# tum-vision/lsd_slam

Measured on AMD Instinct MI355X. Metric: tracked frames/sec (full track+map loop) at 640x480, frames resident in HBM (8-bit upload excluded: value_pcie_inclusive has it), higher is better.
Workload: dtype f32

## Files before the change

lsd_slam_amd/csrc/track_device.hpp:

```cpp
#pragma once
#include "lsdhip_internal.hpp"
#include <type_traits>

template <int CTRL, int ROW_MASK, int BANK_MASK>
__device__ __forceinline__ float dpp_f(float v) {
  return __builtin_bit_cast(float, __builtin_amdgcn_update_dpp(0, __builtin_bit_cast(int, v), CTRL, ROW_MASK, BANK_MASK, true));
}
__device__ __forceinline__ int dpp_max_i(int a, int b) { return a > b ? a : b; }
template <int CTRL, int ROW_MASK, int BANK_MASK>
__device__ __forceinline__ int dpp_i(int v) {
  return __builtin_amdgcn_update_dpp(-1, v, CTRL, ROW_MASK, BANK_MASK, false);
}
template <int CTRL, int ROW_MASK, int BANK_MASK>
__device__ __forceinline__ int dpp_i0(int v) {
  return __builtin_amdgcn_update_dpp(0, v, CTRL, ROW_MASK, BANK_MASK, true);
}
__device__ __forceinline__ int wave_max_to_lane63(int v) {
  int t = dpp_max_i(v, dpp_i<0x111, 0xf, 0xf>(v));
  t = dpp_max_i(t, dpp_i<0x112, 0xf, 0xf>(v));
  t = dpp_max_i(t, dpp_i<0x113, 0xf, 0xf>(v));
  t = dpp_max_i(t, dpp_i<0x114, 0xf, 0xe>(t));
  t = dpp_max_i(t, dpp_i<0x118, 0xf, 0xc>(t));
  t = dpp_max_i(t, dpp_i<0x142, 0xa, 0xf>(t));
  t = dpp_max_i(t, dpp_i<0x143, 0xc, 0xf>(t));
// ... 553 lines not shown
  } else {
    S.level = S.level - 1;
    S.phase = 0;
    set_eval_pose(S, T);
  }
  return false;
}

__device__ __forceinline__ void accumulate_point(const PointOut& o, float (&acc)[RS_END]) {
  acc[RS_M] += 1.f;
  acc[RS_SXX] = __builtin_fmaf(o.c1 * o.c1, o.hw, acc[RS_SXX]);
  acc[RS_SYY] = __builtin_fmaf(o.c2 * o.c2, o.hw, acc[RS_SYY]);
  acc[RS_SX] = __builtin_fmaf(o.c1, o.hw, acc[RS_SX]);
  acc[RS_SY] = __builtin_fmaf(o.c2, o.hw, acc[RS_SY]);
  acc[RS_SW] += o.hw;
  if (o.good) { acc[RS_GOOD] += 1.f; acc[RS_SUMRES2] = __builtin_fmaf(o.res, o.res, acc[RS_SUMRES2]); acc[RS_SUMSIGNED] += o.res; }
  else acc[RS_BAD] += 1.f;
  acc[RS_USAGE] += o.usage;
  acc[RS_WERR] += o.werr;
#pragma unroll
  for (int r = 0; r < 6; r++) {
    float Jw = o.J[r] * o.w;
#pragma unroll
    for (int c = r; c < 6; c++) acc[tri_index(r, c)] = __builtin_fmaf(Jw, o.J[c], acc[tri_index(r, c)]);
  }
  float resw = o.res * o.w;
#pragma unroll
  for (int r = 0; r < 6; r++) acc[RS_B0 + r] = __builtin_fmaf(resw, o.J[r], acc[RS_B0 + r]);
  acc[RS_ERR] = __builtin_fmaf(resw, o.res, acc[RS_ERR]);
}

__device__ __forceinline__ void visit_point(const EvalCtx& a, const PointWarp& q, const PointTexels& t, const float pz, const float I_ref, const float var,
                                            gbyte* mask, const int maskIdx, const int key, float (&acc)[RS_END], int& key0, int& key1, int& key2) {
  acc[RS_NREF] += 1.f;
  if (!q.in_image) { if (mask) mask[maskIdx] = 0; return; }
  PointOut o;
  eval_finish(a, q, t, pz, I_ref, var, o);
  if (mask) mask[maskIdx] = o.good ? 1 : 0;
  top3_insert(key, key0, key1, key2);
  accumulate_point(o, acc);
}

enum { TAIL_WORDS = 29, TAIL_KEY = 31, TAIL_STRIDE = 32, TAIL_ROWS = 3 };
__device__ __forceinline__ void tail_row(const PointOut& o, float* row) {
  row[0] = o.werr;
  int k = 1;
#pragma unroll
  for (int rr = 0; rr < 6; rr++) {
    const float Jw = o.J[rr] * o.w;
#pragma unroll
    for (int cc = rr; cc < 6; cc++) row[k++] = Jw * o.J[cc];
  }
  const float resw = o.res * o.w;
#pragma unroll
  for (int rr = 0; rr < 6; rr++) row[k++] = resw * o.J[rr];
  row[k++] = resw * o.res;
}
__device__ __forceinline__ void tail_row_from_sums(const float (&acc)[RS_END], float* row) {
  row[0] = acc[RS_WERR];
#pragma unroll
  for (int k = 0; k < 21; k++) row[1 + k] = acc[RS_A0 + k];
#pragma unroll
  for (int k = 0; k < 6; k++) row[22 + k] = acc[RS_B0 + k];
  row[28] = acc[RS_ERR];
}
__device__ __forceinline__ int tail_word(const int col) {
  return (col == RS_WERR) ? 0 : ((col >= RS_A0 && col < RS_B0) ? 1 + col - RS_A0 : ((col >= RS_B0 && col < RS_ERR) ? 22 + col - RS_B0 : (col == RS_ERR ? 28 : -1)));
}
__device__ __forceinline__ float tail_drop(float s, const int M, const int nsub, const int word, const float (*sub)[TAIL_STRIDE]) {
  int need = M & 3;
  if (need > nsub) need = nsub;
  const float sub0 = sub[0][word < 0 ? 0 : word], sub1 = sub[1][word < 0 ? 0 : word], sub2 = sub[2][word < 0 ? 0 : word];
  if (word >= 0) {
    if (need > 0) s -= sub0;
    if (need > 1) s -= sub1;
    if (need > 2) s -= sub2;
  }
  return s;
}

struct TailCandidate {
  int key = -1, x = 0, y = 0;
  float var = 0.f, id = 1.f, img = 0.f;
  __device__ __forceinline__ void request(const EvalCtx& a, const int k) {
    key = k;
    if (k < 0) return;
    x = k / a.h; y = k - x * a.h;
    const int ci = __mul24(y, a.w) + x;
    var = a.kf_idepthVar[ci]; id = a.kf_idepth[ci]; img = a.kf_image[ci];
  }
};

template <int STRIDE, int RRUN>
__device__ __forceinline__ float slice_sum(const float* s_red, const int k, const int slice) {
  const float* row = s_red + k * STRIDE;
  const int j0 = slice * RRUN;
  float v[RRUN];
#pragma unroll
  for (int j = 0; j < RRUN; j++) v[j] = row[j0 + j];
  float s = 0.f;
#pragma unroll
  for (int j = 0; j < RRUN; j++) s += (j0 + j < STRIDE - 1) ? v[j] : 0.f;
  return s;
}

template <class Posed>
__device__ __forceinline__ void ctx_set_pose(EvalCtx& a, const Posed& p) {
#pragma unroll
  for (int i = 0; i < 9; i++) a.R[i] = p.R[i];
#pragma unroll
  for (int i = 0; i < 3; i++) a.t[i] = p.t[i];
}
__device__ __forceinline__ void make_ctx_dev(const TrackJob& jobr, const TrackState& S, int level, EvalCtx& a) {
  const TrackJob* job = &jobr;
  const TrackLevel& L = job->lv[level];
  a.kf_idepth = (gfloat*)L.kf_idepth; a.kf_idepthVar = (gfloat*)L.kf_idepthVar; a.kf_image = (gfloat*)L.kf_image; a.fr_grad = (gfloat*)L.fr_grad;
  a.pts_pos = (gfloat*)L.pts_pos; a.pts_colvar = (gfloat*)L.pts_colvar; a.npts = L.npts; a.w = L.w; a.h = L.h;
  a.fx = L.fx; a.fy = L.fy; a.cx = L.cx; a.cy = L.cy; a.fxi = L.fxi; a.fyi = L.fyi; a.cxi = L.cxi; a.cyi = L.cyi;
  ctx_set_pose(a, S);
  a.aff_a = S.aff_a; a.aff_b = S.aff_b;
  a.cameraPixelNoise2 = job->cameraPixelNoise2; a.var_weight = job->var_weight; a.huber_half = job->huber_half;
}

template <int N>
__device__ __forceinline__ void copy_words(void* dst, const void* src, int tid, int nthreads) {
  const unsigned* s = (const unsigned*)src;
  unsigned* d = (unsigned*)dst;
  for (int i = tid; i < N; i += nthreads) d[i] = s[i];
}

__device__ __forceinline__ int xcd_tile(int b, int nb) { return (nb & 7) == 0 ? (b & 7) * (nb >> 3) + (b >> 3) : b; }


struct TrialRecord {
  float inc[6];
  float pose[7];
  float R[9], t[3];
  float pad_[7];
};
static_assert(sizeof(TrialRecord) == 128 && sizeof(lsdm::SE3fH) == sizeof(float[7]), "a trial record is 32 floats; its pose is a TrackState::Tn");
enum { TRIAL_RECORD_WORDS = offsetof(TrialRecord, pad_) / 4 };
__device__ __forceinline__ float trial_record_word(const TrackState& S, const int i) {
  constexpr int P = offsetof(TrialRecord, pose) / 4, R = offsetof(TrialRecord, R) / 4, T = offsetof(TrialRecord, t) / 4;
  return i < P ? S.inc[i] : (i < R ? ((const float*)&S.Tn)[i - P] : (i < T ? S.R[i - R] : S.t[i - T]));
}
__device__ __forceinline__ void trial_record_adopt(TrackState& S, const TrialRecord& rec, const int lane) {
  if (lane < 6) S.inc[lane] = rec.inc[lane];
  if (lane < 7) ((float*)&S.Tn)[lane] = rec.pose[lane];
  if (lane < 9) S.R[lane] = rec.R[lane];
  if (lane < 3) S.t[lane] = rec.t[lane];
}
__device__ __forceinline__ int trials_at(const TrackSpec& spec, const int level) { return (spec.specC > 1 && spec.trials[level] > 1) ? spec.trials[level] : 1; }

#define RS_COLS 44
struct TrackScratch {
  float* sums;
  int4* topkey;
  float* topval;
  int max_rows;
  int cmax;
  TrialRecord* recs;
#ifdef LSD_PHASE_TRACE
  unsigned long long* trace;
#endif
};
```

lsd_slam_amd/csrc/tracker.hip:

```cpp
#include <atomic>
#include <chrono>
#include "track_device.hpp"
#include "reposition_plan.hpp"

#ifdef LSD_PHASE_TRACE
#define PHASE_MARK(k) do { if (trOn_ && threadIdx.x == 0) tr_[k] = clock64(); } while (0)
#define LSD_TRACE_WORDS 32
#define TRACE_PARAMS , const bool trOn_, unsigned long long* const tr_
#define TRACE_ARGS , trOn_, tr_
#define TRACE_PUT(rec, who, k, v) do { if (trOn_ && threadIdx.x == (who)) (rec)[k] = (unsigned long long)(v); } while (0)
#define TRACE_LM_REC (trOn_ ? tr_ : nullptr)
__device__ __forceinline__ unsigned long long* trace_open(unsigned long long* trace, const bool mine, unsigned long long** s_trp) {
  if (!mine) return trace;
  const unsigned long long n = trace[0];
  trace[0] = n + 1;
  unsigned long long* tr_ = trace + 1 + (n % 4096) * LSD_TRACE_WORDS;
  for (int k = 0; k < LSD_TRACE_WORDS; k++) tr_[k] = 0;
  tr_[8] = wall_clock64();
  tr_[24] = (unsigned long long)gridDim.x; tr_[25] = (unsigned long long)gridDim.y;
  *s_trp = tr_;
  return tr_;
}
#else
#define PHASE_MARK(k) do { } while (0)
#define TRACE_PARAMS
#define TRACE_ARGS
#define TRACE_PUT(rec, who, k, v) do { } while (0)
#define TRACE_LM_REC nullptr
#endif

#ifdef LSD_DEVTOOLS
#define LAUNCH_LOG(exitCode, pendingIn, ncandIn, pcUsed) do { \
    if (!BATCH && MODE == TS_FUSED && blockIdx.x == 0 && threadIdx.x == 0 && spec.dbgLog && spec.seq != 0) { \
      int* lg_ = spec.dbgLog + ((spec.seq & 0xFFF) * 16); \
      lg_[0] = spec.seq; lg_[1] = (exitCode); lg_[2] = parity | (first << 1) | (spec.last << 2); lg_[3] = lvlIn_; lg_[4] = (pendingIn); lg_[5] = (ncandIn); \
      lg_[6] = (pcUsed); lg_[7] = S.level; lg_[8] = S.numEvaluations; lg_[9] = S.numLaunches; lg_[10] = S.done; lg_[11] = S.phase; lg_[12] = S.incTry; \
      lg_[13] = S.ncand; lg_[14] = S.pending; lg_[15] = numLaunchesIn_; } } while (0)
#else
#define LAUNCH_LOG(exitCode, pendingIn, ncandIn, pcUsed) do { } while (0)
#endif

enum { TS_FUSED = 0, TS_LM = 1, TS_EVAL = 2 };
__device__ __forceinline__ void track_state_begin(TrackState& S, const TrackJob& job, const int tid) {
  if (tid == 0) {
    S.T = job.T0;
    set_eval_pose(S, job.T0);
    S.aff_a = job.aff_a0; S.aff_b = job.aff_b0; S.aff_a_lastIt = job.aff_a0; S.aff_b_lastIt = job.aff_b0;
    S.lastErr = 0; S.LM_lambda = 0; S.last_residual = 0;
    S.level = job.topLevel; S.iteration = 0; S.incTry = 0; S.phase = 0; S.pending = 0;
    S.done = 0; S.diverged = 0; S.numEvaluations = 0; S.numWarpUpdates = 0;
    S.pointUsage = 0; S.goodCount = 0; S.badCount = 0; S.meanRes = 0;
    S.bytes = 0;
    for (int l = 0; l < LSD_LEVELS; l++) S.levelEvals[l] = 0;
    S.ncand = 1; S.lastCand = 0; S.numLaunches = 0;
  }
  if (tid < 36) S.A[tid] = 0;
  if (tid < 6) { S.b[tid] = 0; S.inc[tid] = 0; }
}

struct StepAddr {
  const float *sums_in, *topval_in;
  float *sums_out, *topval_out;
  const int4* topkey_in; int4* topkey_out;
  const TrialRecord* recs_in;
  TrialRecord* recs_out;
  int max_rows, cmax;
};
template <bool BATCH, int MODE>
__device__ __forceinline__ StepAddr step_addr(const TrackScratch& sc, const int parity) {
  const size_t rows = (size_t)sc.max_rows, cm = (size_t)sc.cmax, job0 = BATCH ? (size_t)blockIdx.y * 2 * cm : 0;
  const size_t in = job0 + (size_t)parity * cm, out = job0 + (size_t)(MODE == TS_EVAL ? parity : 1 - parity) * cm;
  constexpr size_t TAIL = TAIL_ROWS * TAIL_STRIDE;
  return {sc.sums + in * RS_COLS * rows, sc.topval + in * rows * TAIL, sc.sums + out * RS_COLS * rows, sc.topval + out * rows * TAIL,
          sc.topkey + in * rows, sc.topkey + out * rows, sc.recs + in, sc.recs + out, sc.max_rows, sc.cmax};
}

struct StepRole { int cand, bx; bool leader, leaves; };
template <bool BATCH, int MODE>
__device__ __forceinline__ void step_role(StepRole& r, const TrackJob& job, const TrackSpec& spec, const TrackState& S) {
  const int lvlPending = S.level;
  if (MODE == TS_FUSED) {
    const int nbl = job.lv[lvlPending].nblocks;
    const int tr = trials_at(spec, lvlPending);
    r.cand = (int)blockIdx.x / nbl; r.bx = (int)blockIdx.x - r.cand * nbl;
    const bool needTrial = S.pending ? r.cand < tr : r.cand == 0;
    const bool needNext = S.pending && lvlPending > job.lastLevel && (int)blockIdx.x < job.lv[lvlPending - 1].nblocks;
    r.leaves = !r.leader && !needTrial && !needNext;
  }
  if (BATCH && MODE == TS_LM) {
    r.cand = (int)blockIdx.x; r.bx = 0;
    r.leaves = !r.leader && !(S.pending && r.cand < trials_at(spec, lvlPending));
  }
  if (BATCH && MODE == TS_EVAL) {
    const int nbl = job.lv[lvlPending].nblocks;
    r.cand = (int)blockIdx.x / nbl; r.bx = (int)blockIdx.x - r.cand * nbl;
  }
}

constexpr int STRIP_CHMAX = 8;
__device__ __forceinline__ void strip_request(const TrackLevel& L, const int tile_, const int wave, const int lane, int& cntv, unsigned (&ow)[STRIP_CHMAX]) {
  const int px = L.w * L.h;
  const int base_ = tile_ * L.tilePx;
  const int b0_ = base_ >> 8;
  const int mblk_ = (min(base_ + L.tilePx, px) - base_ + 255) >> 8;
  const gbyte* offs = (const gbyte*)L.kf_refBlk;
  const __attribute__((address_space(1))) int* cnts = (const __attribute__((address_space(1))) int*)(offs + ((size_t)((px + 255) >> 8) << 8));
  cntv = lane < mblk_ ? cnts[b0_ + lane] : 0;
#pragma unroll
  for (int c = 0; c < STRIP_CHMAX; c++) {
    const int blk = c * 4 + wave;
    ow[c] = blk < mblk_ ? *(const __attribute__((address_space(1))) unsigned*)(offs + ((size_t)(b0_ + blk) << 8) + (lane << 2)) : 0u;
  }
}

typedef float (*TailTable)[TAIL_ROWS][TAIL_STRIDE];
template <int KROWS>
__device__ __forceinline__ void top3_of_keys(const int4 (&kv)[KROWS], const int lane, int (&keys)[3], int (&src)[3]) {
  Top3Payload top;
#pragma unroll
  for (int q = 0; q < KROWS; q++) {
    const int e = (lane + 64 * q) * 3;
    const int ks[3] = {kv[q].x, kv[q].y, kv[q].z};
#pragma unroll
    for (int rr = 0; rr < 3; rr++) top.insert(ks[rr], e + rr);
  }
#pragma unroll
  for (int r = 0; r < 3; r++) keys[r] = top.take(src[r]);
}
template <int KROWS>
__device__ __forceinline__ void tail_two(const TrackJob& job, const TrackState& S, const int level, const int nb, const StepAddr& A, const TrialRecord* s_rec,
                                         const TailTable s_subT, int* const s_nsubT, const int ca, const int cb, const int lane) {
  const int max_rows = A.max_rows;
  const int cbb = cb < 0 ? ca : cb;
  const int4* tka = A.topkey_in + (size_t)ca * max_rows;
  const int4* tkb = A.topkey_in + (size_t)cbb * max_rows;
  int4 kva[KROWS], kvb[KROWS];
#pragma unroll
  for (int q = 0; q < KROWS; q++) {
    const int row = lane + 64 * q;
    const int4 ka = tka[row < max_rows ? row : 0];
    const int4 kb = tkb[row < max_rows ? row : 0];
    kva[q] = row < nb ? ka : make_int4(-1, -1, -1, -1);
    kvb[q] = row < nb ? kb : make_int4(-1, -1, -1, -1);
  }
  const bool single = job.lv[level].singlePass != 0 || job.lv[level].tilePx > 0;
  const int j = lane & 31, rj = lane >> 5;
  int keysA[3], srcA[3], keysB[3], srcB[3];
  float a0 = 0.f, a2 = 0.f, b0 = 0.f, b2 = 0.f;
  auto request = [&](const int c, const int (&keys)[3], const int (&src)[3], float& v0, float& v2) {
    const float* tv = A.topval_in + (size_t)c * max_rows * (TAIL_ROWS * TAIL_STRIDE);
    if (keys[rj] >= 0) v0 = tv[(size_t)src[rj] * TAIL_STRIDE + j];
    if (rj == 0 && keys[2] >= 0) v2 = tv[(size_t)src[2] * TAIL_STRIDE + j];
  };
  auto deliver = [&](const int c, const int (&keys)[3], const float v0, const float v2) {
    if (keys[rj] >= 0) s_subT[c][rj][j] = v0;
    if (rj == 0 && keys[2] >= 0) s_subT[c][2][j] = v2;
  };
  top3_of_keys(kva, lane, keysA, srcA);
  if (single && j < TAIL_WORDS) request(ca, keysA, srcA, a0, a2);
  if (cb >= 0) {
    top3_of_keys(kvb, lane, keysB, srcB);
    if (single && j < TAIL_WORDS) request(cb, keysB, srcB, b0, b2);
  }
  if (lane == 0) {
    s_nsubT[ca] = (keysA[0] >= 0) + (keysA[1] >= 0) + (keysA[2] >= 0);
    if (cb >= 0) s_nsubT[cb] = (keysB[0] >= 0) + (keysB[1] >= 0) + (keysB[2] >= 0);
  }
  if (single) {
    if (j < TAIL_WORDS) {
      deliver(ca, keysA, a0, a2);
      if (cb >= 0) deliver(cb, keysB, b0, b2);
    }
  } else {
    const bool second = lane >= 3;
    const int r = second ? lane - 3 : lane;
    const int c = second ? cb : ca;
    int key = -1;
    if (lane < 6 && c >= 0) key = second ? (r == 0 ? keysB[0] : (r == 1 ? keysB[1] : keysB[2])) : (r == 0 ? keysA[0] : (r == 1 ? keysA[1] : keysA[2]));
    if (key >= 0) {
      EvalCtx a;
      make_ctx_dev(job, S, level, a);
      if (c > 0) ctx_set_pose(a, s_rec[c]);
      const int idx = (a.npts >= 0) ? key : ((key / a.h) + (key % a.h) * a.w);
      float px, py, pz, I_ref, var;
      int maskIdx;
      fetch_point(a, idx, px, py, pz, I_ref, var, maskIdx);
      PointOut o;
      eval_point(a, px, py, pz, I_ref, var, o);
      tail_row(o, s_subT[c][r]);
    }
  }
}
static_assert(TAIL_STRIDE == 32 && TAIL_KEY == 31, "a tail row is eight 16-byte words; the key is the last word of the eighth");
template <int NQ>
__device__ __forceinline__ void tail_rows_pick(const float4 (&v)[NQ], const int nf4, float (*const sub)[TAIL_STRIDE], int* const nsubOut, const int lane) {
  Top3Payload top;
#pragma unroll
  for (int q = 0; q < NQ; q++) {
    const int f = q * 64 + lane;
    top.insert(((lane & 7) == 7 && f < nf4) ? __float_as_int(v[q].w) : -1, f >> 3);
  }
  int nsub = 0;
#pragma unroll
  for (int r = 0; r < 3; r++) {
    int row;
    const int m = top.take(row);
    if (m >= 0) {
      nsub++;
      const int qsel = row >> 3;
#pragma unroll
      for (int q = 0; q < NQ; q++) {
        if (q == qsel) {
          float4 w4 = v[q];
          asm volatile("" : "+v"(w4.x), "+v"(w4.y), "+v"(w4.z), "+v"(w4.w));
          if ((lane >> 3) == (row & 7)) *(float4*)&sub[r][(lane & 7) * 4] = w4;
        }
      }
    }
  }
  if (lane == 0) *nsubOut = nsub;
}
template <int NQ>
__device__ __forceinline__ void tail_rows(const int nb, const StepAddr& A, const TailTable s_subT, int* const s_nsubT, const int ca, const int cb, const int lane) {
  const int cbb = cb < 0 ? ca : cb;
  const float4* ta = (const float4*)(A.topval_in + (size_t)ca * A.max_rows * (TAIL_ROWS * TAIL_STRIDE));
  const float4* tb = (const float4*)(A.topval_in + (size_t)cbb * A.max_rows * (TAIL_ROWS * TAIL_STRIDE));
  const int nf4 = nb * (TAIL_ROWS * TAIL_STRIDE / 4);
  float4 va[NQ], vb[NQ];
#pragma unroll
  for (int q = 0; q < NQ; q++) {
    const int f = q * 64 + lane;
    va[q] = ta[f < nf4 ? f : 0];
    vb[q] = tb[f < nf4 ? f : 0];
  }
  tail_rows_pick(va, nf4, s_subT[ca], &s_nsubT[ca], lane);
  if (cb >= 0) tail_rows_pick(vb, nf4, s_subT[cb], &s_nsubT[cb], lane);
}
template <bool BATCH, int WAVES>
__device__ __forceinline__ void gather_tails(const TrackJob& job, const TrackState& S, const int level, const int nb, const int ncandPending, const StepAddr& A,
                                             const TrialRecord* s_rec, const TailTable s_subT, int* const s_nsubT, const int wave, const int lane) {
  const int ca = WAVES - 1 - wave;
  const int cb = ca + WAVES < ncandPending ? ca + WAVES : -1;
  if (ca < ncandPending) {
    if (BATCH && job.lv[level].tilePx > 0 && nb <= 24) {
      if (nb <= 5) tail_rows<2>(nb, A, s_subT, s_nsubT, ca, cb, lane);
      else if (nb <= 13) tail_rows<5>(nb, A, s_subT, s_nsubT, ca, cb, lane);
      else tail_rows<9>(nb, A, s_subT, s_nsubT, ca, cb, lane);
    } else if (nb <= 128) tail_two<2>(job, S, level, nb, A, s_rec, s_subT, s_nsubT, ca, cb, lane);
    else tail_two<5>(job, S, level, nb, A, s_rec, s_subT, s_nsubT, ca, cb, lane);
  }
}

constexpr int SUM_NSLOT = 16;
constexpr int SUM_QMAX = 20;
typedef float (*SumTable)[SUM_NSLOT][RS_COLS];
template <int Q, int NT>
__device__ __forceinline__ void colsum(const float4* p, const size_t trialStrideF4, const int nb, const int ncandPending, const int base,
                                       const int slot, const int c4, const bool sumLane, const SumTable s_sumT) {
  constexpr int NSLOT = SUM_NSLOT;
  const int K = (nb + NSLOT - 1) / NSLOT;
  float4 v[NT][Q];
#pragma unroll
  for (int c = 0; c < NT; c++) {
    const int pc = base + c < ncandPending ? base + c : ncandPending - 1;
    const float4* pp = p + (size_t)pc * trialStrideF4;
#pragma unroll
    for (int q = 0; q < Q; q++) {
      const int r = slot + NSLOT * q;
      v[c][q] = pp[(size_t)(r < nb ? r : slot) * (RS_COLS / 4)];
    }
  }
#pragma unroll
  for (int c = 0; c < NT; c++) {
    float4 a4 = make_float4(0.f, 0.f, 0.f, 0.f);
#pragma unroll
    for (int q = 0; q < Q; q++) {
      const bool live = q < K && slot + NSLOT * q < nb;
      a4.x += live ? v[c][q].x : 0.f;
      a4.y += live ? v[c][q].y : 0.f;
      a4.z += live ? v[c][q].z : 0.f;
      a4.w += live ? v[c][q].w : 0.f;
    }
    if (sumLane && base + c < ncandPending) *(float4*)&s_sumT[base + c][slot][c4 * 4] = a4;
  }
}
template <int TRIALS_MAX>
__device__ __forceinline__ void column_sums(const StepAddr& A, const int nb, const int ncandPending, const int t, const SumTable s_sumT) {
  constexpr int NSLOT = SUM_NSLOT, QMAX = SUM_QMAX;
  const int slot_ = t / (RS_COLS / 4); const bool sumLane = slot_ < NSLOT;
  const int slot = sumLane ? slot_ : 0, c4 = sumLane ? t - slot_ * (RS_COLS / 4) : 0;
  const int K = (nb + NSLOT - 1) / NSLOT;
  const float4* p = (const float4*)A.sums_in + c4;
  const size_t trialStrideF4 = (size_t)RS_COLS * A.max_rows / 4;
  if (ncandPending == 1) {
    if (K <= 2) colsum<2, 1>(p, trialStrideF4, nb, ncandPending, 0, slot, c4, sumLane, s_sumT);
    else if (K <= 5) colsum<5, 1>(p, trialStrideF4, nb, ncandPending, 0, slot, c4, sumLane, s_sumT);
    else if (K <= 10) colsum<10, 1>(p, trialStrideF4, nb, ncandPending, 0, slot, c4, sumLane, s_sumT);
    else colsum<QMAX, 1>(p, trialStrideF4, nb, ncandPending, 0, slot, c4, sumLane, s_sumT);
  } else if (K <= 2) colsum<2, TRIALS_MAX>(p, trialStrideF4, nb, ncandPending, 0, slot, c4, sumLane, s_sumT);
  else if (K <= 5) colsum<5, TRIALS_MAX>(p, trialStrideF4, nb, ncandPending, 0, slot, c4, sumLane, s_sumT);
  else if (K <= 10) { for (int base = 0; base < ncandPending; base += 3) colsum<10, 3>(p, trialStrideF4, nb, ncandPending, base, slot, c4, sumLane, s_sumT); }
  else { for (int base = 0; base < ncandPending; base++) colsum<QMAX, 1>(p, trialStrideF4, nb, ncandPending, base, slot, c4, sumLane, s_sumT); }
}
template <int TRIALS_MAX>
struct FinishTables {
  enum { WORDS = TRIALS_MAX * (SUM_NSLOT * RS_COLS + TAIL_ROWS * TAIL_STRIDE + 1) };
  SumTable sum; TailTable sub; int* nsub;
  __device__ __forceinline__ explicit FinishTables(float* buf)
      : sum((SumTable)buf), sub((TailTable)(buf + TRIALS_MAX * SUM_NSLOT * RS_COLS)), nsub((int*)(buf + TRIALS_MAX * (SUM_NSLOT * RS_COLS + TAIL_ROWS * TAIL_STRIDE))) {}
};
__device__ __forceinline__ float slot_total(const SumTable s_sumT, const int c, const int col) {
  float s = s_sumT[c][0][col];
#pragma unroll
  for (int k = 1; k < SUM_NSLOT; k++) s += s_sumT[c][k][col];
  return s;
}

__device__ __forceinline__ int pick_trial(TrackState& S, const LmPar& par, const int level, const int ncandPending, const SumTable s_sumT, const TailTable s_subT,
                                          const int* s_nsubT, const TrialRecord* s_rec, const int tid) {
  if (ncandPending <= 1) return 0;
  const int c = tid < ncandPending ? tid : 0;
  const int Mc = (int)slot_total(s_sumT, c, RS_M);
  const float ws = tail_drop(slot_total(s_sumT, c, RS_WERR), Mc, s_nsubT[c], tail_word(RS_WERR), s_subT[c]);
  const float werrc = lm_werr(ws, Mc);
  const float incdot = inc_norm2(c == 0 ? S.inc : s_rec[c].inc);
  const bool stop = Mc < par.minWarped || werrc < S.lastErr || !(incdot > par.stepSizeMin);
  const unsigned long long sm = __ballot(stop && tid < ncandPending);
  const int pc = sm ? (int)__ffsll((long long)sm) - 1 : ncandPending - 1;
  if (pc > 0) {
    float lam = S.LM_lambda;
    const int it0 = S.incTry;
    for (int j = 0; j < pc; j++) lam = lm_lambda_fail(lam, it0 + j, par.lambdaFailFac);
    const float skipped = eval_bytes(slot_total(s_sumT, 0, RS_NREF), par);
    const float bytes0 = S.bytes;
    const int ne0 = S.numEvaluations, le0 = S.levelEvals[level];
    float bytes1 = bytes0;
    for (int j = 0; j < pc; j++) bytes1 = bytes1 + skipped;
    S.LM_lambda = lam;
    S.incTry = it0 + pc;
    S.numEvaluations = ne0 + pc;
    if (tid == 0) S.levelEvals[level] = le0 + pc;
    S.bytes = bytes1;
    trial_record_adopt(S, s_rec[pc], tid);
  }
  return pc;
}
__device__ __forceinline__ float finish_totals(const SumTable s_sumT, const TailTable s_subT, const int* s_nsubT, const int pc, const int tid) {
  const int M = (int)slot_total(s_sumT, pc, RS_M);
  const float s = tid < RS_END ? slot_total(s_sumT, pc, tid) : 0.f;
  return tail_drop(s, M, s_nsubT[pc], tail_word(tid), s_subT[pc]);
}
template <int BLOCK>
__device__ __forceinline__ void copy_side_mask(const TrackJob& job, const TrackState& S, const TrackSpec& spec, const int level, const int bx, const int nb, const int tid) {
  const uint8_t* side = spec.wasGoodSide + (size_t)(S.lastCand - 1) * spec.maskStride;
  EvalCtx a;
  make_ctx_dev(job, S, level, a);
  const int work = a.npts >= 0 ? a.npts : a.w * a.h;
  for (int i = bx * BLOCK + tid; i < work; i += nb * BLOCK) {
    float px, py, pz, I_ref, var;
    int maskIdx;
    if (fetch_point(a, i, px, py, pz, I_ref, var, maskIdx) && maskIdx >= 0) job.wasGood[maskIdx] = side[maskIdx];
  }
}

template <int BLOCK>
__device__ __forceinline__ void eval_strip(const EvalCtx& a, const int tilePx, const int tile, const int work, const int cntv, const unsigned (&ow)[STRIP_CHMAX],
                                           unsigned* const s_list , gbyte* const wasGood, float (&acc)[RS_END], int& key0, int& key1, int& key2,
                                           const int tid TRACE_PARAMS) {
  const int wave = tid >> 6, lane = tid & 63;
  const int base = tile * tilePx;
  const int stripEnd = min(base + tilePx, work);
  const int b0 = base >> 8;
  const int mblk = (stripEnd - base + 255) >> 8;
  const float inv_w = 1.0f / (float)a.w;
  const int incl = wave_scan32(cntv);
  const int total = __builtin_amdgcn_readlane(incl, 31);
  const int waveU = __builtin_amdgcn_readfirstlane(wave);
  PHASE_MARK(20);
#pragma unroll
  for (int c = 0; c < STRIP_CHMAX; c++) {
    const int blk = c * 4 + waveU;
    if (blk < mblk) {
      const int cb = __builtin_amdgcn_readlane(cntv, blk);
      const int pb = __builtin_amdgcn_readlane(incl, blk) - cb;
#pragma unroll
      for (int k = 0; k < 4; k++) {
        const int sl = lane + 64 * k;
        if (sl < cb) s_list[pb + sl] = pixel_xy16(((b0 + blk) << 8) + (int)((ow[c] >> (8 * k)) & 255u), a.w, inv_w);
      }
    }
  }
  __syncthreads();
  PHASE_MARK(21);
// ... 19 lines not shown
      eval_fetch(a, B.q, B.live && B.q.in_image, B.t);
    };
    const int rounds = (total + BLOCK - 1) / BLOCK;
    StA A1, A2;
    StB B0, B1;
    stageA(tid, A1);
    stageB(A1, B0);
    stageA(tid + BLOCK, A1);
    PHASE_MARK(22);
    auto stageC = [&](const StB& B) {
      if (B.live) {
        const int x_ = (int)(B.xy & 0xffffu), y_ = (int)(B.xy >> 16);
        visit_point(a, B.q, B.t, B.pz, B.I_ref, B.var, wasGood, __mul24(y_, a.w) + x_, __mul24(x_, a.h) + y_, acc, key0, key1, key2);
      }
    };
    for (int r = 0; r < rounds; r += 2) {
      stageB(A1, B1);
      stageA(tid + (r + 2) * BLOCK, A2);
      stageC(B0);
      stageB(A2, B0);
      stageA(tid + (r + 3) * BLOCK, A1);
      stageC(B1);
    }
  }
  __syncthreads();
}
__device__ __forceinline__ void eval_groups_of_four(const EvalCtx& a, int i, const int stride, const int work, gbyte* const wasGood, float (&acc)[RS_END],
                                                    int& key0, int& key1, int& key2) {
  const int sy = stride / a.w, sx = stride - sy * a.w;
  int x = i % a.w, y = i / a.w;
  struct Pt { int i, x, y; bool valid; RefPlanes r; float img, pz; PointWarp q; PointTexels t; };
  while (i < work) {
    Pt P[4];
#pragma unroll
    for (int k = 0; k < 4; k++) {
      Pt& p = P[k];
      p.i = i; p.x = x; p.y = y;
      p.valid = i < work;
      const int li = p.valid ? i : 0;
      fetch_request(a, li, p.r);
      p.img = a.kf_image[li];
      i += stride; x += sx; y += sy;
      if (x >= a.w) { x -= a.w; y++; }
    }
#pragma unroll
    for (int k = 0; k < 4; k++) {
      Pt& p = P[k];
      float px = 0.f, py = 0.f;
      p.pz = 1.f;
      p.valid = p.valid && ref_pixel_inside(a, p.x, p.y) && fetch_finish(a, p.x, p.y, p.r, px, py, p.pz);
      eval_warp(a, px, py, p.pz, p.q);
      eval_fetch(a, p.q, p.valid && p.q.in_image, p.t);
    }
#pragma unroll
    for (int k = 0; k < 4; k++) {
      const Pt& p = P[k];
      if (p.valid) visit_point(a, p.q, p.t, p.pz, p.img, p.r.var, wasGood, p.i, p.x * a.h + p.y, acc, key0, key1, key2);
    }
  }
}
__device__ __forceinline__ void eval_plain(const EvalCtx& a, const int i0, const int stride, const int work, gbyte* const wasGood, float (&acc)[RS_END],
                                           int& key0, int& key1, int& key2) {
  for (int i = i0; i < work; i += stride) {
    float px, py, pz, I_ref, var;
    int maskIdx;
    if (fetch_point(a, i, px, py, pz, I_ref, var, maskIdx)) {
      PointWarp q; PointTexels t;
      eval_warp(a, px, py, pz, q);
      if (q.in_image) eval_fetch(a, q, true, t);
      visit_point(a, q, t, pz, I_ref, var, maskIdx >= 0 ? wasGood : nullptr, maskIdx, a.npts >= 0 ? i : (i % a.w) * a.h + (i / a.w), acc, key0, key1, key2);
    }
  }
}

constexpr int RED_NPASS = 1;
constexpr int RED_CPP = (RS_END + RED_NPASS - 1) / RED_NPASS;
template <int BLOCK, bool BATCH, int MODE>
__device__ __forceinline__ void reduce_and_store(const EvalCtx& a, const TrackLevel& L, TrackState& S, const int tile, const float (&acc)[RS_END],
                                                 const int key0, const int key1, const int key2, float* const s_red, float (*const s_sum)[64], int (*const s_wtop)[3],
                                                 int* const s_top, float* const sums_out, int4* const topkey_out, float* const topval_out, const int tid) {
  constexpr int NPASS = RED_NPASS, CPP = RED_CPP;
  constexpr int RSLICE = BLOCK / CPP;
  constexpr int RRUN = (BLOCK + RSLICE - 1) / RSLICE;
  const bool stripRows = BATCH && L.tilePx > 0;
  const bool candLane = tid >= BLOCK - 64 && tid < BLOCK - 61;
  TailCandidate c;
  float cPz = 0.f;
  PointWarp cq; PointTexels ct;
  if (stripRows) {
    block_top3(key0, key1, key2, s_wtop, s_top);
    if (candLane) c.request(a, s_top[tid - (BLOCK - 64)]);
  }
#pragma unroll
  for (int hp = 0; hp < NPASS; hp++) {
    if (hp > 0) __syncthreads();
#pragma unroll
    for (int k = 0; k < CPP; k++)
      if (hp * CPP + k < RS_END) s_red[k * (BLOCK + 1) + tid] = acc[hp * CPP + k];
    __syncthreads();
    if (MODE == TS_FUSED && hp == 0 && tid == 0) { S.pending = 1; S.numLaunches = S.numLaunches + 1; }
    if (stripRows && hp == 0 && candLane && c.key >= 0) {
      float px, py;
      ref_point_at(a, c.x, c.y, c.id, px, py, cPz);
      eval_warp(a, px, py, cPz, cq);
      eval_fetch(a, cq, cq.in_image, ct);
    }
    {
      const int slice = tid / CPP, k = tid - slice * CPP;
      if (slice < RSLICE) s_sum[slice][k] = slice_sum<BLOCK + 1, RRUN>(s_red, k, slice);
    }
    __syncthreads();
    if (stripRows && hp == 0 && candLane) {
      float* row = topval_out + (size_t)(tile * TAIL_ROWS + (tid - (BLOCK - 64))) * TAIL_STRIDE;
      if (c.key >= 0) {
        PointOut o;
        eval_finish(a, cq, ct, cPz, c.img, c.var, o);
        tail_row(o, row);
      }
      ((int*)row)[TAIL_KEY] = c.key;
    }
    if (tid < CPP && hp * CPP + tid < RS_END) {
      float s = s_sum[0][tid];
#pragma unroll
      for (int sl = 1; sl < RSLICE; sl++) s += s_sum[sl][tid];
      sums_out[(size_t)tile * RS_COLS + (hp * CPP + tid)] = s;
    }
  }
  if (!stripRows) block_top3(key0, key1, key2, s_wtop, s_top);
  if (tid == 0) topkey_out[tile] = make_int4(s_top[0], s_top[1], s_top[2], -1);
  if (L.singlePass && key0 >= 0) {
    const int r = key0 == s_top[0] ? 0 : (key0 == s_top[1] ? 1 : (key0 == s_top[2] ? 2 : -1));
    if (r >= 0) tail_row_from_sums(acc, topval_out + (size_t)(tile * TAIL_ROWS + r) * TAIL_STRIDE);
  }
}

#ifdef LSD_ORDER_CHECK
__device__ __forceinline__ void order_check_totals(const TrackSpec& spec, const float s, const int pc, const int tid) {
  unsigned hv = tid < RS_END ? __float_as_uint(s) * (2654435761u * (unsigned)(tid + 1)) : 0u;
  hv += (unsigned)pc * 97u;
  for (int off = 32; off > 0; off >>= 1) hv += __shfl_xor(hv, off);
  if (tid == 0) {
    const unsigned long long slot = 8 + 2 * ((spec.dbgCum / 400ull) % 8192ull);
    __hip_atomic_fetch_min(&spec.dbgCounters[slot], (unsigned long long)hv, __ATOMIC_RELAXED, __HIP_MEMORY_SCOPE_AGENT);
    __hip_atomic_fetch_max(&spec.dbgCounters[slot + 1], (unsigned long long)hv, __ATOMIC_RELAXED, __HIP_MEMORY_SCOPE_AGENT);
  }
}
#endif

__device__ __forceinline__ void warm_job_arguments() {
  typedef const unsigned __attribute__((address_space(4))) cuint;
  cuint* ka = (cuint*)__builtin_amdgcn_kernarg_segment_ptr();
  unsigned warm = 0;
#pragma unroll
  for (int i = 0; i < (int)(sizeof(TrackJob) / 4); i += 32) warm ^= ka[i];
  asm volatile("" ::"s"(warm));
}

template <int BLOCK, bool BATCH, int MODE>
__device__ __forceinline__ void track_step_impl(const TrackJob& jobv, const TrackJob* __restrict__ jobs, TrackState* __restrict__ st2,
                                                TrackScratch sc, TrackSummary* __restrict__ out, int parity, int first, const TrackSpec& spec) {
  const TrackJob& job = BATCH ? jobs[blockIdx.y] : jobv;
  if (!BATCH) warm_job_arguments();
  if (BATCH) { st2 += 2 * (size_t)blockIdx.y; out += blockIdx.y; }
  const StepAddr A = step_addr<BATCH, MODE>(sc, parity);
  constexpr int WAVES = BLOCK / 64, SUMW = WAVES - 1;
  constexpr int NSLICE = (SUMW * 64) / RS_END, CPP = RED_CPP, RSLICE_ = BLOCK / CPP;
  __shared__ TrackState S;
  __shared__ LmShared sh;
  __shared__ LmPar s_par;
  __shared__ float s_sum[(NSLICE > RSLICE_ ? NSLICE : RSLICE_)][64];
  __shared__ __attribute__((aligned(16))) float s_red[CPP * (BLOCK + 1) + 8];
  __shared__ int s_wtop[WAVES][3];
  __shared__ int s_top[3];
  const int tid = threadIdx.x, wave = tid >> 6, lane = tid & 63;
  StepRole role = {0, (int)blockIdx.x, blockIdx.x == 0, false};
  const bool leader = role.leader;
  TrackState* next = st2 + (1 - parity);
  constexpr int TRIALS_MAX = BATCH ? (MODE == TS_EVAL ? 1 : LSD_BATCH_SPEC_MAX) : LSD_SPEC_MAX;
  constexpr bool SPEC_LM = MODE != TS_EVAL;
  static_assert(FinishTables<TRIALS_MAX>::WORDS <= CPP * (BLOCK + 1) + 8, "the finishing phase's tables must fit the reduction buffer");
  const FinishTables<TRIALS_MAX> ft(s_red);
  __shared__ TrialRecord s_rec[TRIALS_MAX];
#ifdef LSD_PHASE_TRACE
  __shared__ unsigned long long* s_trp;
  const bool trOn_ = sc.trace != nullptr && (int)blockIdx.x == (BATCH ? spec.traceWg : 0) && (!BATCH || blockIdx.y == 0);
  unsigned long long* const tr_ = trace_open(sc.trace, trOn_ && tid == 0, &s_trp);
#endif
  PHASE_MARK(0);
  if (!BATCH && MODE == TS_FUSED && !first && !leader && st2[parity].done) return;
  if (!BATCH && MODE == TS_FUSED && leader && tid == 0 && spec.seq != 0) out->seq = spec.seq;
  if (first) {
    track_state_begin(S, job, tid);
  } else {
    copy_words<sizeof(TrackState) / 4>(&S, st2 + parity, tid, BLOCK);
    if (SPEC_LM && A.cmax > 1 && tid < (int)(sizeof(s_rec) / 4)) ((float*)s_rec)[tid] = ((const float*)A.recs_in)[tid < (int)(sizeof(TrialRecord) / 4) * A.cmax ? tid : 0];
  }
  __syncthreads();
  PHASE_MARK(1);
#ifdef LSD_DEVTOOLS
  const int lvlIn_ = S.level, numLaunchesIn_ = S.numLaunches, pendingIn_ = S.pending, ncandIn_ = S.ncand;
#endif
  if (S.done) {
    LAUNCH_LOG(1, pendingIn_, ncandIn_, -1);
    if (MODE != TS_EVAL && leader) { copy_words<sizeof(TrackState) / 4>(next, &S, tid, BLOCK); }
    return;
  }
  const int lvlPending = S.level;
  const int doneWord = (MODE == TS_FUSED && spec.seq != 0) ? (BATCH ? spec.seq : (spec.seq >> 12)) : 1;
  step_role<BATCH, MODE>(role, job, spec, S);
  if (role.leaves) return;
  int cand = role.cand, bx = role.bx;

  int cntv = 0;
  unsigned ow[STRIP_CHMAX];
  bool havePre = false;
  if (BATCH && MODE == TS_FUSED && S.pending && job.lv[lvlPending].tilePx > 0) {
    havePre = cand < trials_at(spec, lvlPending);
    if (havePre) strip_request(job.lv[lvlPending], xcd_tile(bx, job.lv[lvlPending].nblocks), wave, lane, cntv, ow);
  }

  if (MODE != TS_EVAL && S.pending) {
    const int ncandPending = S.ncand < 1 ? 1 : (S.ncand > TRIALS_MAX ? TRIALS_MAX : S.ncand);
    const int level = S.level;
    const int nb = job.lv[level].nblocks;
    if (tid == SUMW * 64 - 1) stage_lm_par(job, level, s_par, trials_at(spec, level));
    if (wave < SUMW) {
      column_sums<TRIALS_MAX>(A, nb, ncandPending, tid, ft.sum);
      TRACE_PUT(tr_, 0, 17, clock64());
    }
    gather_tails<BATCH, WAVES>(job, S, level, nb, ncandPending, A, s_rec, ft.sub, ft.nsub, wave, lane);
    TRACE_PUT(s_trp, SUMW * 64, 18, clock64());
    __syncthreads();
    PHASE_MARK(2);
    if (wave == 0) {
      const int pc = pick_trial(S, s_par, level, ncandPending, ft.sum, ft.sub, ft.nsub, s_rec, tid);
      const float s = finish_totals(ft.sum, ft.sub, ft.nsub, pc, tid);
      if (tid < RS_NUM) sh.tot[tid] = s;
#ifdef LSD_ORDER_CHECK
      if (!BATCH && spec.dbgCounters) order_check_totals(spec, s, pc, tid);
#endif
      PHASE_MARK(3);
      TRACE_PUT(tr_, 0, 19, ncandPending); TRACE_PUT(tr_, 0, 7, pc);
      lm_wave<SPEC_LM>(s_par, S, s, sh, tid, leader ? out : nullptr, TRACE_LM_REC, pc, cand, doneWord);
    }
    __syncthreads();
    PHASE_MARK(4);
    if (S.done) {
      if (!BATCH && MODE == TS_FUSED && S.lastCand > 0 && spec.copyMask != 0 && job.lv[level].writeMask && cand == 0 && bx < nb)
        copy_side_mask<BLOCK>(job, S, spec, level, bx, nb, tid);
      if (leader) copy_words<sizeof(TrackState) / 4>(next, &S, tid, BLOCK);
      LAUNCH_LOG(2, pendingIn_, ncandIn_, S.lastCand);
      return;
    }
    if (cand > 0 && bx == 0 && S.phase == 1 && cand < S.ncand && tid < TRIAL_RECORD_WORDS) ((float*)&A.recs_out[cand])[tid] = trial_record_word(S, tid);
  }

  if (MODE == TS_LM) {
    __syncthreads();
    if (tid == 0) { S.pending = 1; S.numLaunches = S.numLaunches + 1; }
    __syncthreads();
    if (leader) copy_words<sizeof(TrackState) / 4>(next, &S, tid, BLOCK);
    return;
  }

  const int level = S.level;
  const TrackLevel& L = job.lv[level];
  const int nb = L.nblocks;
  if (MODE == TS_FUSED && level != lvlPending) { cand = 0; bx = (int)blockIdx.x; }
  if (bx >= nb || cand >= S.ncand) return;
  const int tile = xcd_tile(bx, nb);
  EvalCtx a;
  make_ctx_dev(job, S, level, a);
  if (BATCH && MODE == TS_EVAL && cand > 0) ctx_set_pose(a, A.recs_in[cand]);
  gbyte* wasGood = (gbyte*)(L.writeMask ? (cand == 0 ? job.wasGood : spec.wasGoodSide + (size_t)(cand - 1) * spec.maskStride) : nullptr);
  const int work = a.npts >= 0 ? a.npts : a.w * a.h;
  float acc[RS_END];
#pragma unroll
  for (int k = 0; k < RS_END; k++) acc[k] = 0.f;
  int key0 = -1, key1 = -1, key2 = -1;
  if (BATCH && L.tilePx > 0) {
    if (!(havePre && level == lvlPending)) strip_request(L, tile, wave, lane, cntv, ow);
    eval_strip<BLOCK>(a, L.tilePx, tile, work, cntv, ow, (unsigned*)s_red , wasGood, acc, key0, key1, key2, tid TRACE_ARGS);
  } else if (!BATCH && L.evalBatch != 0) {
    eval_groups_of_four(a, tile * BLOCK + tid, nb * BLOCK, work, wasGood, acc, key0, key1, key2);
  } else {
    eval_plain(a, tile * BLOCK + tid, nb * BLOCK, work, wasGood, acc, key0, key1, key2);
  }
  PHASE_MARK(5);
  TRACE_PUT(tr_, 0, 10, level); TRACE_PUT(tr_, 0, 11, nb); TRACE_PUT(tr_, 0, 26, lvlPending);
  reduce_and_store<BLOCK, BATCH, MODE>(a, L, S, tile, acc, key0, key1, key2, s_red, s_sum, s_wtop, s_top, A.sums_out + (size_t)cand * RS_COLS * A.max_rows,
                                       A.topkey_out + (size_t)cand * A.max_rows, A.topval_out + (size_t)cand * A.max_rows * (TAIL_ROWS * TAIL_STRIDE), tid);
  if (MODE == TS_FUSED && leader) copy_words<sizeof(TrackState) / 4>(next, &S, tid, BLOCK);
  if (MODE == TS_FUSED && leader && tid == 0 && spec.last != 0) out->exhausted = spec.seq;
  LAUNCH_LOG(3, pendingIn_, ncandIn_, S.lastCand);
  PHASE_MARK(6);
  TRACE_PUT(tr_, 0, 9, wall_clock64());
}

template <int BLOCK, bool BATCH, int MODE = TS_FUSED>
__global__ __launch_bounds__(BLOCK) void k_track_step(TrackJob jobv, const TrackJob* __restrict__ jobs, TrackState* __restrict__ st2,
                                                       TrackScratch sc, TrackSummary* __restrict__ out, int parity, int first, TrackSpec spec) {
#ifdef LSD_ORDER_CHECK
  if (!BATCH && spec.dbgCounters && threadIdx.x == 0) {
    const unsigned long long fin = __hip_atomic_load(&spec.dbgCounters[0], __ATOMIC_RELAXED, __HIP_MEMORY_SCOPE_AGENT);
    if (fin < spec.dbgCum) {
      __hip_atomic_fetch_add(&spec.dbgCounters[1], 1ull, __ATOMIC_RELAXED, __HIP_MEMORY_SCOPE_AGENT);
      __hip_atomic_fetch_max(&spec.dbgCounters[2], spec.dbgCum - fin, __ATOMIC_RELAXED, __HIP_MEMORY_SCOPE_AGENT);
    }
  }
#endif
  track_step_impl<BLOCK, BATCH, MODE>(jobv, jobs, st2, sc, out, parity, first, spec);
#ifdef LSD_ORDER_CHECK
  __syncthreads();
  if (!BATCH && spec.dbgCounters && threadIdx.x == 0) __hip_atomic_fetch_add(&spec.dbgCounters[0], 1ull, __ATOMIC_RELEASE, __HIP_MEMORY_SCOPE_AGENT);
// ... 1739 lines not shown
```

Before: 5714.

## Precompute tail rows in reduce for all paths and overlap tail key loads with column sums

The producer-side reduction now always runs block_top3 first and, for non-single-pass levels, evaluates the top-3 candidate points itself, using listed point positions when available. This removes the consumer-side fallback that re-evaluated tail points in gather. The consumer merges column sums and tail gathering into one routine. For small block counts it issues the tail key loads before the column sums so their latency overlaps, and it splits column_sums into short and many-row template variants to shrink the code. It also widens the trace record for per-wave marks. The risk is extra work per tile in the reduce kernel and higher register pressure from the keys held across the sums.

```diff
diff --git a/lsd_slam_amd/csrc/track_device.hpp b/lsd_slam_amd/csrc/track_device.hpp
--- a/lsd_slam_amd/csrc/track_device.hpp
+++ b/lsd_slam_amd/csrc/track_device.hpp
@@ -659,12 +659,23 @@
 struct TailCandidate {
   int key = -1, x = 0, y = 0;
   float var = 0.f, id = 1.f, img = 0.f;
+  float px = 0.f, py = 0.f, pz = 1.f;
   __device__ __forceinline__ void request(const EvalCtx& a, const int k) {
     key = k;
     if (k < 0) return;
     x = k / a.h; y = k - x * a.h;
     const int ci = __mul24(y, a.w) + x;
     var = a.kf_idepthVar[ci]; id = a.kf_idepth[ci]; img = a.kf_image[ci];
+  }
+  __device__ __forceinline__ void request_listed(const EvalCtx& a, const int k) {
+    key = k;
+    if (k < 0) return;
+    px = a.pts_pos[3 * k]; py = a.pts_pos[3 * k + 1]; pz = a.pts_pos[3 * k + 2];
+    img = a.pts_colvar[2 * k]; var = a.pts_colvar[2 * k + 1];
+  }
+  __device__ __forceinline__ void point(const EvalCtx& a, float& qx, float& qy, float& qz) const {
+    if (a.npts >= 0) { qx = px; qy = py; qz = pz; }
+    else ref_point_at(a, x, y, id, qx, qy, qz);
   }
 };
 
diff --git a/lsd_slam_amd/csrc/tracker.hip b/lsd_slam_amd/csrc/tracker.hip
--- a/lsd_slam_amd/csrc/tracker.hip
+++ b/lsd_slam_amd/csrc/tracker.hip
@@ -5,9 +5,11 @@
 
 #ifdef LSD_PHASE_TRACE
 #define PHASE_MARK(k) do { if (trOn_ && threadIdx.x == 0) tr_[k] = clock64(); } while (0)
-#define LSD_TRACE_WORDS 32
+#define LSD_TRACE_WORDS 48
 #define TRACE_PARAMS , const bool trOn_, unsigned long long* const tr_
 #define TRACE_ARGS , trOn_, tr_
+#define TRACE_ARGS_WG , trOn_, s_trp
+#define WAVE_MARK(e) do { if (trOn_ && (threadIdx.x & 63) == 0) tr_[32 + 4 * (e) + (threadIdx.x >> 6)] = clock64(); } while (0)
 #define TRACE_PUT(rec, who, k, v) do { if (trOn_ && threadIdx.x == (who)) (rec)[k] = (unsigned long long)(v); } while (0)
 #define TRACE_LM_REC (trOn_ ? tr_ : nullptr)
 __device__ __forceinline__ unsigned long long* trace_open(unsigned long long* trace, const bool mine, unsigned long long** s_trp) {
@@ -25,6 +27,8 @@
 #define PHASE_MARK(k) do { } while (0)
 #define TRACE_PARAMS
 #define TRACE_ARGS
+#define TRACE_ARGS_WG
+#define WAVE_MARK(e) do { } while (0)
 #define TRACE_PUT(rec, who, k, v) do { } while (0)
 #define TRACE_LM_REC nullptr
 #endif
@@ -128,22 +132,30 @@
   for (int r = 0; r < 3; r++) keys[r] = top.take(src[r]);
 }
 template <int KROWS>
-__device__ __forceinline__ void tail_two(const TrackJob& job, const TrackState& S, const int level, const int nb, const StepAddr& A, const TrialRecord* s_rec,
-                                         const TailTable s_subT, int* const s_nsubT, const int ca, const int cb, const int lane) {
+struct TailKeys { int4 a[KROWS], b[KROWS]; };
+template <int KROWS>
+__device__ __forceinline__ void tail_request_keys(const StepAddr& A, const int ca, const int cb, const int lane, TailKeys<KROWS>& k) {
   const int max_rows = A.max_rows;
-  const int cbb = cb < 0 ? ca : cb;
   const int4* tka = A.topkey_in + (size_t)ca * max_rows;
-  const int4* tkb = A.topkey_in + (size_t)cbb * max_rows;
-  int4 kva[KROWS], kvb[KROWS];
+  const int4* tkb = A.topkey_in + (size_t)(cb < 0 ? ca : cb) * max_rows;
 #pragma unroll
   for (int q = 0; q < KROWS; q++) {
     const int row = lane + 64 * q;
-    const int4 ka = tka[row < max_rows ? row : 0];
-    const int4 kb = tkb[row < max_rows ? row : 0];
-    kva[q] = row < nb ? ka : make_int4(-1, -1, -1, -1);
-    kvb[q] = row < nb ? kb : make_int4(-1, -1, -1, -1);
-  }
-  const bool single = job.lv[level].singlePass != 0 || job.lv[level].tilePx > 0;
+    k.a[q] = tka[row < max_rows ? row : 0];
+    k.b[q] = tkb[row < max_rows ? row : 0];
+  }
+}
+template <int KROWS>
+__device__ __forceinline__ void tail_finish(const int nb, const StepAddr& A, const TailTable s_subT, int* const s_nsubT, const int ca, const int cb, const int lane,
+                                            const TailKeys<KROWS>& k TRACE_PARAMS) {
+  const int max_rows = A.max_rows;
+  int4 kva[KROWS], kvb[KROWS];
+#pragma unroll
+  for (int q = 0; q < KROWS; q++) {
+    const bool live = lane + 64 * q < nb;
+    kva[q] = live ? k.a[q] : make_int4(-1, -1, -1, -1);
+    kvb[q] = live ? k.b[q] : make_int4(-1, -1, -1, -1);
+  }
   const int j = lane & 31, rj = lane >> 5;
   int keysA[3], srcA[3], keysB[3], srcB[3];
   float a0 = 0.f, a2 = 0.f, b0 = 0.f, b2 = 0.f;
@@ -157,38 +169,19 @@
     if (rj == 0 && keys[2] >= 0) s_subT[c][2][j] = v2;
   };
   top3_of_keys(kva, lane, keysA, srcA);
-  if (single && j < TAIL_WORDS) request(ca, keysA, srcA, a0, a2);
+  WAVE_MARK(1);
+  if (j < TAIL_WORDS) request(ca, keysA, srcA, a0, a2);
   if (cb >= 0) {
     top3_of_keys(kvb, lane, keysB, srcB);
-    if (single && j < TAIL_WORDS) request(cb, keysB, srcB, b0, b2);
+    if (j < TAIL_WORDS) request(cb, keysB, srcB, b0, b2);
   }
   if (lane == 0) {
     s_nsubT[ca] = (keysA[0] >= 0) + (keysA[1] >= 0) + (keysA[2] >= 0);
     if (cb >= 0) s_nsubT[cb] = (keysB[0] >= 0) + (keysB[1] >= 0) + (keysB[2] >= 0);
   }
-  if (single) {
-    if (j < TAIL_WORDS) {
-      deliver(ca, keysA, a0, a2);
-      if (cb >= 0) deliver(cb, keysB, b0, b2);
-    }
-  } else {
-    const bool second = lane >= 3;
-    const int r = second ? lane - 3 : lane;
-    const int c = second ? cb : ca;
-    int key = -1;
-    if (lane < 6 && c >= 0) key = second ? (r == 0 ? keysB[0] : (r == 1 ? keysB[1] : keysB[2])) : (r == 0 ? keysA[0] : (r == 1 ? keysA[1] : keysA[2]));
-    if (key >= 0) {
-      EvalCtx a;
-      make_ctx_dev(job, S, level, a);
-      if (c > 0) ctx_set_pose(a, s_rec[c]);
-      const int idx = (a.npts >= 0) ? key : ((key / a.h) + (key % a.h) * a.w);
-      float px, py, pz, I_ref, var;
-      int maskIdx;
-      fetch_point(a, idx, px, py, pz, I_ref, var, maskIdx);
-      PointOut o;
-      eval_point(a, px, py, pz, I_ref, var, o);
-      tail_row(o, s_subT[c][r]);
-    }
+  if (j < TAIL_WORDS) {
+    deliver(ca, keysA, a0, a2);
+    if (cb >= 0) deliver(cb, keysB, b0, b2);
   }
 }
 static_assert(TAIL_STRIDE == 32 && TAIL_KEY == 31, "a tail row is eight 16-byte words; the key is the last word of the eighth");
@@ -236,21 +229,6 @@
   tail_rows_pick(va, nf4, s_subT[ca], &s_nsubT[ca], lane);
   if (cb >= 0) tail_rows_pick(vb, nf4, s_subT[cb], &s_nsubT[cb], lane);
 }
-template <bool BATCH, int WAVES>
-__device__ __forceinline__ void gather_tails(const TrackJob& job, const TrackState& S, const int level, const int nb, const int ncandPending, const StepAddr& A,
-                                             const TrialRecord* s_rec, const TailTable s_subT, int* const s_nsubT, const int wave, const int lane) {
-  const int ca = WAVES - 1 - wave;
-  const int cb = ca + WAVES < ncandPending ? ca + WAVES : -1;
-  if (ca < ncandPending) {
-    if (BATCH && job.lv[level].tilePx > 0 && nb <= 24) {
-      if (nb <= 5) tail_rows<2>(nb, A, s_subT, s_nsubT, ca, cb, lane);
-      else if (nb <= 13) tail_rows<5>(nb, A, s_subT, s_nsubT, ca, cb, lane);
-      else tail_rows<9>(nb, A, s_subT, s_nsubT, ca, cb, lane);
-    } else if (nb <= 128) tail_two<2>(job, S, level, nb, A, s_rec, s_subT, s_nsubT, ca, cb, lane);
-    else tail_two<5>(job, S, level, nb, A, s_rec, s_subT, s_nsubT, ca, cb, lane);
-  }
-}
-
 constexpr int SUM_NSLOT = 16;
 constexpr int SUM_QMAX = 20;
 typedef float (*SumTable)[SUM_NSLOT][RS_COLS];
@@ -284,7 +262,8 @@
     if (sumLane && base + c < ncandPending) *(float4*)&s_sumT[base + c][slot][c4 * 4] = a4;
   }
 }
-template <int TRIALS_MAX>
+constexpr int SUM_SHORT_ROWS = 5 * SUM_NSLOT;
+template <int TRIALS_MAX, bool MANY>
 __device__ __forceinline__ void column_sums(const StepAddr& A, const int nb, const int ncandPending, const int t, const SumTable s_sumT) {
   constexpr int NSLOT = SUM_NSLOT, QMAX = SUM_QMAX;
   const int slot_ = t / (RS_COLS / 4); const bool sumLane = slot_ < NSLOT;
@@ -292,15 +271,19 @@
   const int K = (nb + NSLOT - 1) / NSLOT;
   const float4* p = (const float4*)A.sums_in + c4;
   const size_t trialStrideF4 = (size_t)RS_COLS * A.max_rows / 4;
-  if (ncandPending == 1) {
-    if (K <= 2) colsum<2, 1>(p, trialStrideF4, nb, ncandPending, 0, slot, c4, sumLane, s_sumT);
-    else if (K <= 5) colsum<5, 1>(p, trialStrideF4, nb, ncandPending, 0, slot, c4, sumLane, s_sumT);
-    else if (K <= 10) colsum<10, 1>(p, trialStrideF4, nb, ncandPending, 0, slot, c4, sumLane, s_sumT);
-    else colsum<QMAX, 1>(p, trialStrideF4, nb, ncandPending, 0, slot, c4, sumLane, s_sumT);
-  } else if (K <= 2) colsum<2, TRIALS_MAX>(p, trialStrideF4, nb, ncandPending, 0, slot, c4, sumLane, s_sumT);
-  else if (K <= 5) colsum<5, TRIALS_MAX>(p, trialStrideF4, nb, ncandPending, 0, slot, c4, sumLane, s_sumT);
-  else if (K <= 10) { for (int base = 0; base < ncandPending; base += 3) colsum<10, 3>(p, trialStrideF4, nb, ncandPending, base, slot, c4, sumLane, s_sumT); }
-  else { for (int base = 0; base < ncandPending; base++) colsum<QMAX, 1>(p, trialStrideF4, nb, ncandPending, base, slot, c4, sumLane, s_sumT); }
+  if (!MANY) {
+    if (ncandPending == 1) {
+      if (K <= 2) colsum<2, 1>(p, trialStrideF4, nb, ncandPending, 0, slot, c4, sumLane, s_sumT);
+      else colsum<5, 1>(p, trialStrideF4, nb, ncandPending, 0, slot, c4, sumLane, s_sumT);
+    } else if (K <= 2) colsum<2, TRIALS_MAX>(p, trialStrideF4, nb, ncandPending, 0, slot, c4, sumLane, s_sumT);
+    else colsum<5, TRIALS_MAX>(p, trialStrideF4, nb, ncandPending, 0, slot, c4, sumLane, s_sumT);
+  } else {
+    if (ncandPending == 1) {
+      if (K <= 10) colsum<10, 1>(p, trialStrideF4, nb, ncandPending, 0, slot, c4, sumLane, s_sumT);
+      else colsum<QMAX, 1>(p, trialStrideF4, nb, ncandPending, 0, slot, c4, sumLane, s_sumT);
+    } else if (K <= 10) { for (int base = 0; base < ncandPending; base += 3) colsum<10, 3>(p, trialStrideF4, nb, ncandPending, base, slot, c4, sumLane, s_sumT); }
+    else { for (int base = 0; base < ncandPending; base++) colsum<QMAX, 1>(p, trialStrideF4, nb, ncandPending, base, slot, c4, sumLane, s_sumT); }
+  }
 }
 template <int TRIALS_MAX>
 struct FinishTables {
@@ -309,6 +292,43 @@
   __device__ __forceinline__ explicit FinishTables(float* buf)
       : sum((SumTable)buf), sub((TailTable)(buf + TRIALS_MAX * SUM_NSLOT * RS_COLS)), nsub((int*)(buf + TRIALS_MAX * (SUM_NSLOT * RS_COLS + TAIL_ROWS * TAIL_STRIDE))) {}
 };
+template <bool BATCH, int WAVES, int TRIALS_MAX>
+__device__ __forceinline__ void gather_sums_and_tails(const TrackJob& job, const int level, const int nb, const int ncandPending, const StepAddr& A,
+                                                      const FinishTables<TRIALS_MAX>& ft, const int tid TRACE_PARAMS) {
+  const int wave = __builtin_amdgcn_readfirstlane(tid >> 6), lane = tid & 63;
+  const int ca = WAVES - 1 - wave;
+  const int cb = ca + WAVES < ncandPending ? ca + WAVES : -1;
+  const bool sums = wave < WAVES - 1, tails = ca < ncandPending;
+  const bool stripRows = BATCH && job.lv[level].tilePx > 0 && nb <= 24;
+  if (nb <= SUM_SHORT_ROWS) {
+    TailKeys<2> k;
+    if (tails && !stripRows) tail_request_keys(A, ca, cb, lane, k);
+    if (sums) {
+      column_sums<TRIALS_MAX, false>(A, nb, ncandPending, tid, ft.sum);
+      WAVE_MARK(0);
+      TRACE_PUT(tr_, 0, 17, clock64());
+    }
+    if (tails) {
+      if (!stripRows) tail_finish(nb, A, ft.sub, ft.nsub, ca, cb, lane, k TRACE_ARGS);
+      else if (nb <= 5) tail_rows<2>(nb, A, ft.sub, ft.nsub, ca, cb, lane);
+      else if (nb <= 13) tail_rows<5>(nb, A, ft.sub, ft.nsub, ca, cb, lane);
+      else tail_rows<9>(nb, A, ft.sub, ft.nsub, ca, cb, lane);
+    }
+  } else {
+    if (sums) {
+      column_sums<TRIALS_MAX, true>(A, nb, ncandPending, tid, ft.sum);
+      WAVE_MARK(0);
+      TRACE_PUT(tr_, 0, 17, clock64());
+    }
+    if (tails) {
+      TailKeys<5> k;
+      tail_request_keys(A, ca, cb, lane, k);
+      tail_finish(nb, A, ft.sub, ft.nsub, ca, cb, lane, k TRACE_ARGS);
+    }
+  }
+  WAVE_MARK(2);
+  TRACE_PUT(tr_, (WAVES - 1) * 64, 18, clock64());
+}
 __device__ __forceinline__ float slot_total(const SumTable s_sumT, const int c, const int col) {
   float s = s_sumT[c][0][col];
 #pragma unroll
@@ -494,14 +514,20 @@
   constexpr int NPASS = RED_NPASS, CPP = RED_CPP;
   constexpr int RSLICE = BLOCK / CPP;
   constexpr int RRUN = (BLOCK + RSLICE - 1) / RSLICE;
-  const bool stripRows = BATCH && L.tilePx > 0;
+  const bool candRows = (BATCH && L.tilePx > 0) || !L.singlePass;
   const bool candLane = tid >= BLOCK - 64 && tid < BLOCK - 61;
   TailCandidate c;
   float cPz = 0.f;
   PointWarp cq; PointTexels ct;
-  if (stripRows) {
-    block_top3(key0, key1, key2, s_wtop, s_top);
-    if (candLane) c.request(a, s_top[tid - (BLOCK - 64)]);
+  block_top3(key0, key1, key2, s_wtop, s_top);
+  if (candRows && candLane) {
+    if (a.npts >= 0) c.request_listed(a, s_top[tid - (BLOCK - 64)]);
+    else c.request(a, s_top[tid - (BLOCK - 64)]);
+  }
+  if (tid == 0) topkey_out[tile] = make_int4(s_top[0], s_top[1], s_top[2], -1);
+  if (L.singlePass && key0 >= 0) {
+    const int r = key0 == s_top[0] ? 0 : (key0 == s_top[1] ? 1 : (key0 == s_top[2] ? 2 : -1));
+    if (r >= 0) tail_row_from_sums(acc, topval_out + (size_t)(tile * TAIL_ROWS + r) * TAIL_STRIDE);
   }
 #pragma unroll
   for (int hp = 0; hp < NPASS; hp++) {
@@ -511,9 +537,9 @@
       if (hp * CPP + k < RS_END) s_red[k * (BLOCK + 1) + tid] = acc[hp * CPP + k];
     __syncthreads();
     if (MODE == TS_FUSED && hp == 0 && tid == 0) { S.pending = 1; S.numLaunches = S.numLaunches + 1; }
-    if (stripRows && hp == 0 && candLane && c.key >= 0) {
+    if (candRows && hp == 0 && candLane && c.key >= 0) {
       float px, py;
-      ref_point_at(a, c.x, c.y, c.id, px, py, cPz);
+      c.point(a, px, py, cPz);
       eval_warp(a, px, py, cPz, cq);
       eval_fetch(a, cq, cq.in_image, ct);
     }
@@ -522,7 +548,7 @@
       if (slice < RSLICE) s_sum[slice][k] = slice_sum<BLOCK + 1, RRUN>(s_red, k, slice);
     }
     __syncthreads();
-    if (stripRows && hp == 0 && candLane) {
+    if (candRows && hp == 0 && candLane) {
       float* row = topval_out + (size_t)(tile * TAIL_ROWS + (tid - (BLOCK - 64))) * TAIL_STRIDE;
       if (c.key >= 0) {
         PointOut o;
@@ -537,12 +563,6 @@
       for (int sl = 1; sl < RSLICE; sl++) s += s_sum[sl][tid];
       sums_out[(size_t)tile * RS_COLS + (hp * CPP + tid)] = s;
     }
-  }
-  if (!stripRows) block_top3(key0, key1, key2, s_wtop, s_top);
-  if (tid == 0) topkey_out[tile] = make_int4(s_top[0], s_top[1], s_top[2], -1);
-  if (L.singlePass && key0 >= 0) {
-    const int r = key0 == s_top[0] ? 0 : (key0 == s_top[1] ? 1 : (key0 == s_top[2] ? 2 : -1));
-    if (r >= 0) tail_row_from_sums(acc, topval_out + (size_t)(tile * TAIL_ROWS + r) * TAIL_STRIDE);
   }
 }
 
@@ -636,12 +656,7 @@
     const int level = S.level;
     const int nb = job.lv[level].nblocks;
     if (tid == SUMW * 64 - 1) stage_lm_par(job, level, s_par, trials_at(spec, level));
-    if (wave < SUMW) {
-      column_sums<TRIALS_MAX>(A, nb, ncandPending, tid, ft.sum);
-      TRACE_PUT(tr_, 0, 17, clock64());
-    }
-    gather_tails<BATCH, WAVES>(job, S, level, nb, ncandPending, A, s_rec, ft.sub, ft.nsub, wave, lane);
-    TRACE_PUT(s_trp, SUMW * 64, 18, clock64());
+    gather_sums_and_tails<BATCH, WAVES, TRIALS_MAX>(job, level, nb, ncandPending, A, ft, tid TRACE_ARGS_WG);
     __syncthreads();
     PHASE_MARK(2);
     if (wave == 0) {
```

After: 5763, median of 6. About the same (+0.9%).
